# zuston/TonY

Measured on AMD Instinct MI355X. Metric: images/sec (whole node) Inception-v3 TF-PS, higher is better.
Workload: dtype bf16

## Files before the change

tony_amd/ops/csrc/conv.hip:

```cpp
#include <atomic>
#include <algorithm>
#include <cstdlib>
#include <type_traits>

#include "igemm.h"

using namespace tony;
using namespace tony::mfma;
using namespace tony::glds;

namespace tony {
int run_band(const Gather& g, const void* B, void* C, int64_t ldc, int64_t N, int epi, float* st, int64_t sstride,
             hipStream_t stream);
}

namespace {

__device__ __forceinline__ uint4 gather16(const Gather& g, const RowState& rs, const TapPos& t, int toff) {
  const int iy = rs.iy0 + g.sign * t.r, ix = rs.ix0 + g.sign * t.s;
  if (rs.ok && t.r < g.R && static_cast<unsigned>(iy) < static_cast<unsigned>(g.Hs) &&
      static_cast<unsigned>(ix) < static_cast<unsigned>(g.Ws))
    return *reinterpret_cast<const uint4*>(rs.base + toff);
  return make_uint4(0, 0, 0, 0);
}
// ... 602 lines not shown
  if (stats == nullptr) {
    stats = bnr.dsum;
    sstride = bnr.sstride;
  }
  float* st = stats + shard_off(blockIdx.x, sstride);
#pragma unroll
  for (int c = 0; c < D::CB; ++c)
#pragma unroll
    for (int r = 0; r < 4; ++r) {
      float a = ssum[c][r], q = ssq[c][r];
#pragma unroll
      for (int o = 1; o < 16; o <<= 1) {
        a += __shfl_xor(a, o, 64);
        q += __shfl_xor(q, o, 64);
      }
      if ((lane & 15) == 0) {
        atomicAdd(st + c * 16 + kq * 4 + r, a);
        atomicAdd(st + CO + c * 16 + kq * 4 + r, q);
      }
    }
}

int run_direct(const Gather& g, const void* B, void* C, int64_t ldc, int64_t N, int epi, float* st, int64_t sstride,
               hipStream_t stream, const BnRed& bnr = BnRed{}) {
  const bool f32 = (epi & 8) != 0;
  if (g.R != 3 || g.S != 3 || g.sh != 1 || g.sw != 1 || (epi & 22) || (ldc % 4) || g.halo_images <= 0 ||
      (reinterpret_cast<uintptr_t>(C) & (f32 ? 15 : 7)) || (reinterpret_cast<uintptr_t>(B) & 15) ||
      (f32 && bnr.z != nullptr))
    return -3;
  const auto launch = [&](auto cs, auto co, auto tw, auto f32c) -> int {
    constexpr int CS = decltype(cs)::value, CO = decltype(co)::value, TW = decltype(tw)::value;
    constexpr bool F32 = decltype(f32c)::value;
    using D = DirectCfg<CS, CO, TW>;
    const void* fn = reinterpret_cast<const void*>(&conv_direct_kernel<CS, CO, TW, F32>);
    static int per_cu = 0;
    if (per_cu == 0) {
      if (D::kLds > 65536 &&
          hipFuncSetAttribute(fn, hipFuncAttributeMaxDynamicSharedMemorySize, static_cast<int>(D::kLds)) != hipSuccess)
        return -3;
      if (hipOccupancyMaxActiveBlocksPerMultiprocessor(&per_cu, fn, kThreads, D::kLds) != hipSuccess || per_cu <= 0)
        per_cu = -1;
    }
    if (per_cu < 0) return -3;
    int dev = 0, cus = 0;
    if (hipGetDevice(&dev) != hipSuccess || hipDeviceGetAttribute(&cus, hipDeviceAttributeMultiprocessorCount, dev) !=
                                                hipSuccess)
      return -3;
    const int tiles_x = ceil_div(g.OW, TW), tiles_y = ceil_div(g.OH, kDirH);
    const int64_t ntiles = static_cast<int64_t>(g.halo_images) * tiles_x * tiles_y;
    if (ntiles > 0x7fffffff) return -2;
    const int grid = static_cast<int>(std::min<int64_t>(ntiles, static_cast<int64_t>(per_cu) * cus));
    conv_direct_kernel<CS, CO, TW, F32><<<grid, kThreads, D::kLds, stream>>>(
        g, static_cast<const uint16_t*>(B), static_cast<uint16_t*>(C), ldc, st, sstride, tiles_x, tiles_y,
        static_cast<int>(ntiles), bnr);
    TONY_LAUNCH_CHECK();
    return 0;
  };
  using I = std::integral_constant<int, 32>;
  using I64 = std::integral_constant<int, 64>;
  using I96 = std::integral_constant<int, 96>;
  using I16 = std::integral_constant<int, 16>;
  using BF = std::false_type;
  if (f32) {
    if (g.Cs == 96 && N == 32) return launch(I96{}, I{}, I{}, std::true_type{});
    if (g.Cs == 96 && N == 64) return launch(I96{}, I64{}, I16{}, std::true_type{});
    return -3;
  }
  if (g.Cs == 32 && N == 32) return launch(I{}, I{}, I{}, BF{});
  if (g.Cs == 32 && N == 64) return launch(I{}, I64{}, I16{}, BF{});
  if (g.Cs == 64 && N == 32) return launch(I64{}, I{}, I16{}, BF{});
  if (g.Cs == 64 && N == 64) return launch(I64{}, I64{}, I16{}, BF{});
  return -3;
}

int run_nt(const Gather& g, const void* B, void* C, int64_t ldc, int64_t M, int64_t N, int flags, float* stats,
           int64_t sstride, hipStream_t stream, const Phase& bph = Phase{}) {
  const int epi = flags & 31;
  if ((epi & 1) && (epi & 2)) return -1;
  if ((epi & 3) && stats == nullptr) return -1;
  if ((epi & 16) && ((epi & 3) || bph.bnr.z != nullptr)) return -1;
  float* st = stats;
  const int v = (flags >> 8) & 0xff;
  if (((flags >> 16) & 15) && !(v >= kGldsFirst && v < kGldsFirst + kNumGlds)) return -3;
  if (((epi & 24) && v == kHaloVariant) || ((epi & 16) && v == kDirectVariant)) return -3;
  if (v == kHaloVariant) return bph.bnr.z != nullptr ? -3 : run_halo(g, B, C, ldc, N, epi, st, sstride, stream);
  if (v == kBandVariant) return bph.bnr.z != nullptr ? -3 : run_band(g, B, C, ldc, N, epi, st, sstride, stream);
  if (v == kDirectVariant) return run_direct(g, B, C, ldc, N, epi, st, sstride, stream, bph.bnr);
  if (v >= kGldsFirst && v < kGldsFirst + kNumGlds)
    return bph.bnr.z != nullptr ? -3
                                : run_glds(g, B, g.K, C, ldc, M, N, epi, st, sstride, v, stream, RowMap{}, BTaps{},
                                           (flags >> 16) & 15);
  if (v >= kNumNtVariants) return -1;
  if (v == 0) {
    const int64_t bn = pick_bn(N, 192);
    return bn <= 64 ? launch_nt_bm<256>(g, B, C, ldc, M, N, st, sstride, epi, bn, stream, bph)
                    : launch_nt_bm<128>(g, B, C, ldc, M, N, st, sstride, epi, bn, stream, bph);
  }
  const int64_t bn = pick_bn(N, kNtVariants[v].cap);
  switch (kNtVariants[v].bm) {
    case 64: return launch_nt_bm<64>(g, B, C, ldc, M, N, st, sstride, epi, bn, stream, bph);
    case 128: return launch_nt_bm<128>(g, B, C, ldc, M, N, st, sstride, epi, bn, stream, bph);
    default: return launch_nt_bm<256>(g, B, C, ldc, M, N, st, sstride, epi, bn, stream, bph);
  }
}

int run_nt_phase(const Gather& g, const void* B, void* C, int64_t ldc, int64_t M, int64_t N, int v, const Phase& ph,
                 hipStream_t stream, int epi = 0) {
  if (v >= kGldsFirst && ph.bnr.z != nullptr) v = 0;
  if (v >= kGldsFirst)
    return run_glds(g, B, static_cast<int64_t>(ph.R) * ph.S * g.Cs, C, ldc, M, N, epi, nullptr, 0, v, stream, ph.rows,
                    BTaps{ph.r0, ph.s0, ph.tsy, ph.tsx, ph.S});
  if (v == kBandVariant) return -3;
  if (v == kHaloVariant || v == kDirectVariant || v >= kNumNtVariants) return -1;
  if (v == 0) {
    const int64_t bn = pick_bn(N, 192);
    return bn <= 64 ? launch_nt_bm<256, true>(g, B, C, ldc, M, N, nullptr, 0, epi, bn, stream, ph)
                    : launch_nt_bm<128, true>(g, B, C, ldc, M, N, nullptr, 0, epi, bn, stream, ph);
  }
  const int64_t bn = pick_bn(N, kNtVariants[v].cap);
  switch (kNtVariants[v].bm) {
    case 64: return launch_nt_bm<64, true>(g, B, C, ldc, M, N, nullptr, 0, epi, bn, stream, ph);
    case 128: return launch_nt_bm<128, true>(g, B, C, ldc, M, N, nullptr, 0, epi, bn, stream, ph);
    default: return launch_nt_bm<256, true>(g, B, C, ldc, M, N, nullptr, 0, epi, bn, stream, ph);
  }
}

constexpr int WTBM = 128;
constexpr int WTBN = 128;

struct MRow {
  int n, oy, ox;
  int64_t m;
  __device__ __forceinline__ void init(int64_t m_, const Gather& g) {
    m = m_;
    const int ohw = g.OH * g.OW;
    n = static_cast<int>(m_ / ohw);
    const int rem = static_cast<int>(m_ - static_cast<int64_t>(n) * ohw);
    oy = rem / g.OW;
    ox = rem - oy * g.OW;
  }
  __device__ __forceinline__ void advance(int dm, const Gather& g) {
    m += dm;
    ox += dm;
    while (ox >= g.OW) {
      ox -= g.OW;
      if (++oy == g.OH) {
        oy = 0;
        ++n;
      }
    }
  }
};

constexpr int WK = 32;

struct WkStep {
  int dx, dy, de;
  int cx, cy, ce;
  int img_y, img_e;
};

struct IncRows {
  int ix[2], iy[2], ie[2];
  int xlim, ylim;
  __device__ __forceinline__ void init(const MRow* mr, const Gather& g, const TapPos& tp) {
    xlim = g.OW * g.sw + g.offw + tp.s;
// ... 832 lines not shown
    case 96: ring == 3 ? go(std::integral_constant<int, 96>{}, I3{}) : go(std::integral_constant<int, 96>{}, I2{}); break;
    default: ring == 3 ? go(std::integral_constant<int, 128>{}, I3{}) : go(std::integral_constant<int, 128>{}, I2{}); break;
  }
  TONY_LAUNCH_CHECK();
  return 0;
}

int wgrad_tbm(int Co) {
  static const bool t96 = [] {
    const char* e = getenv("TONY_WGRAD_TBM96");
    return e == nullptr || e[0] != '0';
  }();
  if (Co <= 32) return 32;
  if (Co <= 64) return 64;
  return t96 && ceil_div(Co, 96) * 96 < ceil_div(Co, 128) * 128 ? 96 : 128;
}

bool bad_geom(int C, int64_t ld, const void* p) {
  return C <= 0 || (C % 8) || (ld % 8) || (reinterpret_cast<uintptr_t>(p) & 15);
}

}

namespace tony {
SplitWs& splitk_ws() {
  static thread_local SplitWs ws;
  return ws;
}
}

TONY_API int tony_splitk_workspace(float* slab, int64_t slab_floats, unsigned* cnt, int64_t ncnt) {
  if (slab_floats < 0 || ncnt < 0 || (reinterpret_cast<uintptr_t>(slab) & 15)) return -1;
  tony::splitk_ws() = tony::SplitWs{slab, slab_floats, cnt, ncnt};
  return 0;
}

int run_x3(Gather g, const void* B, int Cx, void* C, int64_t ldc, int64_t M, int64_t N, int flags, float* stats,
           int64_t sstride, hipStream_t stream) {
  const int v = (flags >> 8) & 0xff;
  if (v < kX3First || v >= kX3First + kNumX3 || Cx % 3 || (Cx / 3) % 8) return -3;
  const int epi = flags & 31;
  if ((epi & 1) && (epi & 2)) return -1;
  if ((epi & 3) && stats == nullptr) return -1;
  if ((epi & 16) && (epi & 3)) return -1;
  const int cp = Cx / 3;
  g.Cs = cp;
  g.K = g.R * g.S * cp;
  return run_glds_x3(g, B, static_cast<int64_t>(g.R) * g.S * Cx, C, ldc, M, N, epi, stats, sstride, v, stream,
                        RowMap{}, BTaps{}, (flags >> 16) & 15, X3Planes{cp, 2 * cp, 3 * cp});
}

TONY_API int tony_conv_fwd(const void* x, int N, int H, int W, int C, int64_t ldx, const void* w, int Co, int R,
                           int S, int sh, int sw, int ph, int pw, void* y, int OH, int OW, int64_t ldy, int flags,
                           float* stats, int64_t sstride, hipStream_t stream) {
  if (bad_geom(C, ldx, x) || (reinterpret_cast<uintptr_t>(w) & 15) || Co <= 0 || R <= 0 || S <= 0 || sstride < 0)
    return -1;
  if (OH != (H + 2 * ph - R) / sh + 1 || OW != (W + 2 * pw - S) / sw + 1 || OH <= 0 || OW <= 0) return -1;
  const int64_t M = static_cast<int64_t>(N) * OH * OW;
  if (M > 0x7fffffff || static_cast<int64_t>(N) * H * W > 0x7fffffff) return -1;
  Gather g{static_cast<const uint16_t*>(x), ldx, H, W, C, OH, OW, R, S, sh, sw, -ph, -pw, 1, R * S * C, N};
  const int v = (flags >> 8) & 0xff;
  if (v >= kX3First && v < kX3First + kNumX3) return run_x3(g, w, C, y, ldy, M, Co, flags, stats, sstride, stream);
  return run_nt(g, w, y, ldy, M, Co, flags, stats, sstride, stream);
}

TONY_API int tony_conv_dgrad(const void* dy, int N, int OH, int OW, int Co, int64_t lddy, const void* wt, int C,
                             int R, int S, int ph, int pw, void* dx, int H, int W, int64_t lddx, int flags,
                             BnRed* bnr, hipStream_t stream) {
  if (bad_geom(Co, lddy, dy) || (reinterpret_cast<uintptr_t>(wt) & 15) || C <= 0) return -1;
  if (OH != H + 2 * ph - R + 1 || OW != W + 2 * pw - S + 1) return -1;
  const int64_t M = static_cast<int64_t>(N) * H * W;
  if (M > 0x7fffffff || static_cast<int64_t>(N) * OH * OW > 0x7fffffff) return -1;
  Gather g{static_cast<const uint16_t*>(dy), lddy, OH, OW, Co, H, W, R, S, 1, 1, ph, pw, -1, R * S * Co, N};
  Phase bph{};
  if (bnr != nullptr) {
    bnr->done = 0;
    if (bnr->z != nullptr) {
      if (bnr->mean == nullptr || bnr->invstd == nullptr || bnr->dsum == nullptr || (bnr->ldz % 8) ||
          (reinterpret_cast<uintptr_t>(bnr->z) & 15) || (C % 8))
        return -1;
      bph.bnr = *bnr;
    }
  }
  const int fl = flags & 0xfff18;
  if ((fl & 16) && bph.bnr.z != nullptr) return -1;
  const int v = (fl >> 8) & 0xff;
  if (v >= kX3First && v < kX3First + kNumX3)
    return bph.bnr.z != nullptr ? -3 : run_x3(g, wt, Co, dx, lddx, M, C, fl, nullptr, 0, stream);
  const int rc = run_nt(g, wt, dx, lddx, M, C, fl, nullptr, 0, stream, bph);
  if (rc == -3 && bph.bnr.z != nullptr)
    return run_nt(g, wt, dx, lddx, M, C, fl, nullptr, 0, stream);
  if (rc == 0 && bph.bnr.z != nullptr) bnr->done = 1;
  return rc;
}

static std::atomic<int>& dgrad_one_launch_flag() {
  static std::atomic<int> on{[] {
    const char* e = std::getenv("TONY_DGRAD_ONE_LAUNCH");
    return (e != nullptr && e[0] == '0') ? 0 : 1;
  }()};
  return on;
}
static bool dgrad_one_launch() { return dgrad_one_launch_flag().load(std::memory_order_relaxed) != 0; }
TONY_API int tony_wgrad_pf(int on) {
  const int prev = wgrad_pf_flag().load();
  if (on >= 0) wgrad_pf_flag().store(on ? 1 : 0);
  return prev;
}

TONY_API int tony_dgrad_one_launch(int on) {
  const int prev = dgrad_one_launch_flag().load();
  if (on >= 0) dgrad_one_launch_flag().store(on ? 1 : 0);
  return prev;
}

TONY_API int tony_conv_dgrad_strided(const void* dy, int N, int OH, int OW, int Co, int64_t lddy, const void* wt,
                                     int C, int R, int S, int sh, int sw, int ph, int pw, void* dx, int H, int W,
                                     int64_t lddx, int flags, BnRed* bnr, hipStream_t stream) {
  if (bad_geom(Co, lddy, dy) || (reinterpret_cast<uintptr_t>(wt) & 15) || C <= 0 || C % 8 || (lddx % 8) ||
      (reinterpret_cast<uintptr_t>(dx) & 15))
    return -1;
  BnRed br{};
  if (bnr != nullptr) {
    bnr->done = 0;
    if (bnr->z != nullptr) {
      if (bnr->mean == nullptr || bnr->invstd == nullptr || bnr->dsum == nullptr || (bnr->ldz % 8) ||
          (reinterpret_cast<uintptr_t>(bnr->z) & 15))
        return -1;
      br = *bnr;
    }
  }
  if (sh < 1 || sw < 1 || sh > 4 || sw > 4 || ph < 0 || pw < 0 || ph >= R || pw >= S) return -1;
  if (OH != (H + 2 * ph - R) / sh + 1 || OW != (W + 2 * pw - S) / sw + 1 || OH <= 0 || OW <= 0) return -1;
  if (static_cast<int64_t>(N) * H * W > 0x7fffffff || static_cast<int64_t>(N) * OH * OW > 0x7fffffff) return -1;
  const int v = (flags >> 8) & 0xff;
  const int acc = flags & 16;
  if (acc && br.z != nullptr) return -1;
  if ((flags >> 16) & 15) return -3;
  const bool one = v >= kGldsFirst && v < kGldsFirst + kNumGlds && br.z == nullptr && sh * sw <= kMaxClasses &&
                   Co % kGldsVariants[v - kGldsFirst].kb == 0 && dgrad_one_launch();
  MultiClass mc{};
  for (int py = 0; py < sh; ++py) {
    for (int px = 0; px < sw; ++px) {
      const int QH = H > py ? (H - py + sh - 1) / sh : 0, QW = W > px ? (W - px + sw - 1) / sw : 0;
      const int64_t M = static_cast<int64_t>(N) * QH * QW;
      if (M == 0) continue;
      const int r0 = (py + ph) % sh, s0 = (px + pw) % sw;
      int Ra = r0 < R ? (R - r0 + sh - 1) / sh : 0, Sb = s0 < S ? (S - s0 + sw - 1) / sw : 0;
      const int cy = (py + ph - r0) / sh, cx = (px + pw - s0) / sw;
      if (Ra == 0 || Sb == 0) {
        if (acc) continue;
        Ra = 0, Sb = 1;
      }
      Gather g{static_cast<const uint16_t*>(dy), lddy, OH, OW, Co, QH, QW, Ra, Sb, 1, 1, cy, cx, -1, Ra * Sb * Co, N};
      Phase phz{R, S, r0, s0, sh, sw, RowMap{}};
      phz.rows.qw = QW;
      phz.rows.qhw = QH * QW;
      phz.rows.W = W;
      phz.rows.HW = H * W;
      phz.rows.sy = sh;
      phz.rows.sx = sw;
      phz.rows.y0 = py;
      phz.rows.x0 = px;
      phz.bnr = br;
      if (one) {
        mc.c[mc.n++] = ClassDesc{g, phz.rows, BTaps{r0, s0, sh, sw, S}, static_cast<int>(M), 0};
        continue;
// ... 109 lines not shown
```

tony_amd/ops/csrc/gemm.hip:

```cpp
#include <type_traits>
#include <cstdlib>

#include "igemm.h"

using namespace tony;
using namespace tony::mfma;
using namespace tony::glds;

namespace {

template <int ROWS>
__device__ __forceinline__ void load_tile(uint4* regs, const uint16_t* __restrict__ G, int64_t ld, int row0,
                                          int nrows, int k0, int K) {
  constexpr int VEC = ROWS * BK / 8 / kThreads;
#pragma unroll
  for (int i = 0; i < VEC; ++i) {
    const int v = threadIdx.x + i * kThreads;
    const int row = v >> 3, ch = v & 7;
    const int gr = row0 + row, gk = k0 + ch * 8;
    if (gr < nrows && gk < K)
      regs[i] = *reinterpret_cast<const uint4*>(G + static_cast<int64_t>(gr) * ld + gk);
    else
      regs[i] = make_uint4(0, 0, 0, 0);
  }
// ... 69 lines not shown
#pragma unroll
        for (int j = 0; j < TN; ++j) acc[i][j] = __builtin_amdgcn_mfma_f32_16x16x32_bf16(af[i], bfr[j], acc[i][j], 0, 0, 0);
    }
    if (more) {
      uint16_t* An = smem + ((kt + 1) & 1) * (BM + BN) * BK;
      store_tile<BM>(An, ra);
      store_tile<BN>(An + BM * BK, rb);
    }
    __syncthreads();
  }

  const bool am = (epi & 32) != 0;
  nt_epilogue<BM, BN, TM, TN>(acc, smem, C, ldc, M, N, m0, n0,
                               (epi & 1) ? stats + shard_off(tm, sstride) : nullptr,
                               (epi & 2) ? stats : nullptr, (epi & 4) != 0, RowMap{}, (epi & 8) != 0,
                               (epi & 48) != 0, am ? reinterpret_cast<const uint16_t*>(stats) : nullptr,
                               am ? reinterpret_cast<const uint8_t*>(sstride) : nullptr);
}

template <int BM, int BN>
int launch(const void* A, int64_t lda, const void* B, int64_t ldb, void* C, int64_t ldc, int64_t M, int64_t N,
           int64_t K, float* stats, int64_t sstride, int epi, hipStream_t stream) {
  const int tiles_m = ceil_div(M, BM), tiles_n = ceil_div(N, BN);
  const int64_t tiles = static_cast<int64_t>(tiles_m) * tiles_n;
  if (tiles > 0x7fffffff) return -2;
  gemm_nt_kernel<BM, BN><<<static_cast<int>(tiles), kThreads, 0, stream>>>(
      static_cast<const uint16_t*>(A), lda, static_cast<const uint16_t*>(B), ldb, static_cast<uint16_t*>(C), ldc,
      static_cast<int>(M), static_cast<int>(N), static_cast<int>(K), stats, sstride, epi, tiles_n);
  TONY_LAUNCH_CHECK();
  return 0;
}

template <int BM>
int launch_bm(const void* A, int64_t lda, const void* B, int64_t ldb, void* C, int64_t ldc, int64_t M, int64_t N,
              int64_t K, float* st, int64_t sstride, int epi, int64_t bn, hipStream_t stream) {
  if constexpr (BM == 256) {
    if (bn <= 32) return launch<256, 32>(A, lda, B, ldb, C, ldc, M, N, K, st, sstride, epi, stream);
    if (bn <= 64) return launch<256, 64>(A, lda, B, ldb, C, ldc, M, N, K, st, sstride, epi, stream);
    return -3;
  } else {
    switch (bn) {
      case 32: return launch<BM, 32>(A, lda, B, ldb, C, ldc, M, N, K, st, sstride, epi, stream);
      case 64: return launch<BM, 64>(A, lda, B, ldb, C, ldc, M, N, K, st, sstride, epi, stream);
      case 96: return launch<BM, 96>(A, lda, B, ldb, C, ldc, M, N, K, st, sstride, epi, stream);
      case 128: return launch<BM, 128>(A, lda, B, ldb, C, ldc, M, N, K, st, sstride, epi, stream);
      case 160: return launch<BM, 160>(A, lda, B, ldb, C, ldc, M, N, K, st, sstride, epi, stream);
      default: return launch<BM, 192>(A, lda, B, ldb, C, ldc, M, N, K, st, sstride, epi, stream);
    }
  }
}

}

TONY_API int tony_gemm_bf16_bnact(const void* A, const void* B, void* C, int64_t M, int64_t N, int64_t K, int64_t lda,
                                  int64_t ldb, int64_t ldc, int flags, float* stats, int64_t sstride, const float* table,
                                  hipStream_t stream) {
  if (M <= 0 || N <= 0 || K <= 0 || sstride < 0 || table == nullptr) return -1;
  if ((K % 8) || (lda % 8) || (ldb % 8) || M > 0x7fffffff || N > 0x7fffffff) return -1;
  if ((reinterpret_cast<uintptr_t>(A) | reinterpret_cast<uintptr_t>(B)) & 15) return -1;
  const int epi = flags & 31;
  if (((epi & 1) && (epi & 2)) || ((epi & 16) && (epi & 3)) || ((epi & 3) && stats == nullptr)) return -1;
  X3Planes xp{};
  xp.atab = table;
  return run_glds(gemm_gather(A, lda, M, K), B, ldb, C, ldc, M, N, epi, stats, sstride, kGldsFirst + 1, stream,
                  RowMap{}, BTaps{}, 0, xp);
}

TONY_API int tony_gemm_bf16(const void* A, const void* B, void* C, int64_t M, int64_t N, int64_t K, int64_t lda,
                            int64_t ldb, int64_t ldc, int flags, float* stats, int64_t sstride, hipStream_t stream) {
  if (M <= 0 || N <= 0 || K <= 0 || sstride < 0) return -1;
  if ((K % 8) || (lda % 8) || (ldb % 8)) return -1;
  if (M > 0x7fffffff || N > 0x7fffffff) return -1;
  if ((reinterpret_cast<uintptr_t>(A) | reinterpret_cast<uintptr_t>(B)) & 15) return -1;
  const int epi = flags & 63;
  if ((epi & 1) && (epi & 2)) return -1;
  if ((epi & 16) && (epi & 3)) return -1;
  if ((epi & 32) && ((epi & 31) || stats == nullptr || sstride == 0 || (ldc % 8) ||
                     (reinterpret_cast<uintptr_t>(stats) & 15)))
    return -1;
  if ((epi & 3) && stats == nullptr) return -1;
  float* st = stats;
  const int v = (flags >> 8) & 0xff;
  if (((flags >> 16) & 15) && !(v >= kGldsFirst && v < kGldsFirst + kNumGlds)) return -3;
  if (v >= kGldsFirst && v < kGldsFirst + kNumGlds)
    return run_glds(gemm_gather(A, lda, M, K), B, ldb, C, ldc, M, N, epi, st, sstride, v, stream, RowMap{}, BTaps{},
                    (flags >> 16) & 15);
  if (v >= kNumNtVariants) return -1;
  if (v == 0) {
    if (N <= 64) return launch<256, 64>(A, lda, B, ldb, C, ldc, M, N, K, st, sstride, epi, stream);
    return launch<128, 128>(A, lda, B, ldb, C, ldc, M, N, K, st, sstride, epi, stream);
  }
  const int64_t bn = pick_bn(N, kNtVariants[v].cap);
  switch (kNtVariants[v].bm) {
    case 64: return launch_bm<64>(A, lda, B, ldb, C, ldc, M, N, K, st, sstride, epi, bn, stream);
    case 128: return launch_bm<128>(A, lda, B, ldb, C, ldc, M, N, K, st, sstride, epi, bn, stream);
    default: return launch_bm<256>(A, lda, B, ldb, C, ldc, M, N, K, st, sstride, epi, bn, stream);
  }
}

namespace {

constexpr int TBM = 128;
constexpr int TBN = 128;

__device__ __forceinline__ void tn_load(uint4* regs, const uint16_t* __restrict__ G, int64_t ld, int64_t m0,
                                        int64_t m1, int c0, int ncols) {
#pragma unroll
  for (int i = 0; i < 2; ++i) {
    const int v = threadIdx.x + i * kThreads;
    const int row = v >> 4, ch = v & 15;
    const int64_t gm = m0 + row;
    const int gc = c0 + ch * 8;
    if (gm < m1 && gc < ncols)
      regs[i] = *reinterpret_cast<const uint4*>(G + gm * ld + gc);
    else
      regs[i] = make_uint4(0, 0, 0, 0);
  }
}

__device__ __forceinline__ void tn_store(uint16_t* lds, const uint4* regs) {
#pragma unroll
  for (int i = 0; i < 2; ++i) {
    const int v = threadIdx.x + i * kThreads;
    const int row = v >> 4, ch = v & 15;
    *reinterpret_cast<uint4*>(lds + tr_off(row, ch)) = regs[i];
  }
}

constexpr int kTnStages = 3;

__global__ __launch_bounds__(kThreads) __attribute__((amdgpu_waves_per_eu(2, 2))) void gemm_tn_glds_kernel(
    const uint16_t* __restrict__ A, int64_t lda, const uint16_t* __restrict__ B, int64_t ldb, int64_t M, int N1,
    int N2, int tiles_n2, int ntiles, int64_t rows_per_split, float* __restrict__ slab, SplitFold fold) {
  constexpr int TILE = TBK * 128, STAGE = 2 * TILE;
  __shared__ __attribute__((aligned(16))) uint16_t smem[kTnStages * STAGE];
  const int wg = xcd_remap(blockIdx.x, gridDim.x);
  const int tile = wg % ntiles, split = wg / ntiles;
  const int t1 = tile / tiles_n2, t2 = tile % tiles_n2;
  const int n1_0 = t1 * TBM, n2_0 = t2 * TBN;
  const int64_t m_begin = static_cast<int64_t>(split) * rows_per_split;
  const int64_t m_end = min(M, m_begin + rows_per_split);
  const int lane = threadIdx.x & 63, wave = threadIdx.x >> 6;
  const int wm = wave >> 1, wn = wave & 1;

  const int r0 = threadIdx.x >> 4;
  const int ch = (threadIdx.x & 15) ^ tr_swz(r0);
  const bool aok = n1_0 + ch * 8 < N1, bok = n2_0 + ch * 8 < N2;
  const uint16_t* ap = A + n1_0 + ch * 8;
  const uint16_t* bp = B + n2_0 + ch * 8;
  int am = static_cast<int>(m_begin) + r0;
  const int mend = static_cast<int>(m_end);
  const uint16_t* apm = ap + (m_begin + r0) * lda;
  const uint16_t* bpm = bp + (m_begin + r0) * ldb;
  const int64_t astep = TBK * lda, bstep = TBK * ldb;
  const uint32_t base = __builtin_amdgcn_readfirstlane(lds_addr(smem) + (4 * wave) * 256);
  constexpr uint32_t kRow16 = 16 * 256, kStageB = STAGE * 2, kTileB = TILE * 2;
  auto issue = [&](int slot) {
    const uint32_t As = base + slot * kStageB, Bs = As + kTileB;
    const void* z = &kZeroChunk;
#pragma unroll
    for (int i = 0; i < 2; ++i) {
      const bool mok = am + 16 * i < mend;
      glds16(aok & mok ? static_cast<const void*>(apm + i * 16 * lda) : z, As + i * kRow16);
      glds16(bok & mok ? static_cast<const void*>(bpm + i * 16 * ldb) : z, Bs + i * kRow16);
    }
    am += TBK;
// ... 197 lines not shown
```

tony_amd/ops/csrc/igemm.h:

```cpp
#pragma once

#include <algorithm>
#include <cstdlib>
#include <tuple>
#include <type_traits>

#include "mfma_common.h"

namespace tony {
struct SplitWs {
  float* slab = nullptr;
  int64_t slab_floats = 0;
  unsigned* cnt = nullptr;
  int64_t ncnt = 0;
};
SplitWs& splitk_ws();
}

namespace tony {
namespace glds {

using namespace tony::mfma;

struct SplitK {
// ... 572 lines not shown
    if (threadIdx.x == 0) {
      for (unsigned spins = 0; __hip_atomic_load(done, __ATOMIC_RELAXED, __HIP_MEMORY_SCOPE_AGENT) < others &&
                               spins < (1u << 24);
           ++spins)
        __builtin_amdgcn_s_sleep(1);
      __hip_atomic_store(cnt, 0u, __ATOMIC_RELAXED, __HIP_MEMORY_SCOPE_AGENT);
      __hip_atomic_store(done, 0u, __ATOMIC_RELAXED, __HIP_MEMORY_SCOPE_AGENT);
    }
    __syncthreads();
    __builtin_amdgcn_fence(__ATOMIC_ACQUIRE, "wavefront");
    f32x4 own[TM][TN];
#pragma unroll
    for (int i = 0; i < TM; ++i)
#pragma unroll
      for (int j = 0; j < TN; ++j) {
        own[i][j] = acc[i][j];
        acc[i][j] = f32x4{0.f, 0.f, 0.f, 0.f};
      }
    for (int c = w_first; c <= w_last; ++c) {
      if (c == w) {
#pragma unroll
        for (int i = 0; i < TM; ++i)
#pragma unroll
          for (int j = 0; j < TN; ++j) acc[i][j] += own[i][j];
        continue;
      }
      const int slot_c = (2 * c + ((static_cast<int64_t>(c) * T / G) >= t0 ? 0 : 1)) * FR;
#pragma unroll
      for (int i = 0; i < TM; ++i)
#pragma unroll
        for (int j = 0; j < TN; ++j)
          acc[i][j] += __builtin_bit_cast(f32x4, __builtin_amdgcn_raw_buffer_load_b128(
                                                     prs, ((slot_c + i * TN + j) * NT + threadIdx.x) * 16, 0, 16));
    }
  }
  const bool am = (epi & 32) != 0;
  nt_epilogue<BM, BN, TM, TN, ST * STAGE, NWM>(acc, smem, C, ldc, M, N, m0, n0,
                                           (epi & 1) ? stats + shard_off(tm, sstride) : nullptr,
                                           (epi & 2) ? stats : nullptr, (epi & 4) != 0, rmap, (epi & 8) != 0,
                                           (epi & 48) != 0, am ? reinterpret_cast<const uint16_t*>(stats) : nullptr,
                                           am ? reinterpret_cast<const uint8_t*>(sstride) : nullptr);
  if constexpr (!(FT & 1)) break;
  }
}

#define TONY_GLDS_PARAMS                                                                                      \
  Gather g, const uint16_t* __restrict__ B, int64_t ldb, uint16_t* __restrict__ C, int64_t ldc, int M, int N,   \
      float* __restrict__ stats, int64_t sstride, int epi, int tiles_n, RowMap rmap, BTaps bt, SplitK sk,       \
      X3Planes xp, MultiClass mc
#define TONY_GLDS_ARGS g, B, ldb, C, ldc, M, N, stats, sstride, epi, tiles_n, rmap, bt, sk, xp, mc
template <int BM, int BN, int ST, int KB, bool UNI, int NWM = 2, bool IL = false, bool X3 = false, bool AT = false,
          bool PF = false, int FT = 0>
__global__ __launch_bounds__(128 * NWM) void conv_glds_kernel(TONY_GLDS_PARAMS) {
  conv_glds_body<BM, BN, ST, KB, UNI, NWM, IL, X3, AT, PF, FT>(TONY_GLDS_ARGS);
}
template <int BM, int BN, int ST, int KB, bool UNI, int NWM, bool IL, int WPE, int FT = 0>
__global__ __launch_bounds__(128 * NWM) __attribute__((amdgpu_waves_per_eu(WPE))) void conv_glds_occ_kernel(
    TONY_GLDS_PARAMS) {
  conv_glds_body<BM, BN, ST, KB, UNI, NWM, IL, false, false, false, FT>(TONY_GLDS_ARGS);
}
#undef TONY_GLDS_PARAMS
#undef TONY_GLDS_ARGS

constexpr int64_t kStreamMaxTiles = 4096;
inline int num_cus_of_current() {
  static int cached[16] = {0};
  int dev = 0;
  if (hipGetDevice(&dev) != hipSuccess || dev < 0 || dev >= 16) return 256;
  if (cached[dev] == 0) {
    int n = 0;
    cached[dev] = hipDeviceGetAttribute(&n, hipDeviceAttributeMultiprocessorCount, dev) == hipSuccess && n > 0 ? n : 256;
  }
  return cached[dev];
}

struct X3Variant {
  int bm, cap, stages, kb, nwm;
};
constexpr int kX3First = 32;
constexpr X3Variant kX3Variants[] = {{256, 128, 2, 32, 4}, {128, 192, 3, 32, 2}, {128, 128, 4, 32, 2},
                                     {128, 128, 2, 64, 2}, {256, 128, 3, 32, 4}, {64, 128, 4, 32, 2}};
constexpr int kNumX3 = sizeof(kX3Variants) / sizeof(kX3Variants[0]);

constexpr int glds_part(int c) { return c <= 4 ? 0 : c <= 8 ? 1 : c <= 13 ? 2 : 3; }

int run_glds(const Gather& g, const void* B, int64_t ldb, void* C, int64_t ldc, int64_t M, int64_t N, int epi,
             float* st, int64_t sstride, int v, hipStream_t stream, RowMap rmap = RowMap{}, BTaps bt = BTaps{},
             int stream_m = 0, X3Planes xp = X3Planes{}, const MultiClass* classes = nullptr);
int run_glds_x3(const Gather& g, const void* B, int64_t ldb, void* C, int64_t ldc, int64_t M, int64_t N, int epi,
                float* st, int64_t sstride, int v, hipStream_t stream, RowMap rmap, BTaps bt, int stream_m,
                X3Planes xp);
template <bool XF, int PART>
int run_glds_part(const Gather& g, const void* B, int64_t ldb, void* C, int64_t ldc, int64_t M, int64_t N, int epi,
                  float* st, int64_t sstride, int v, hipStream_t stream, RowMap rmap, BTaps bt, int stream_m,
                  X3Planes xp, const MultiClass* classes);

}
}
```

tony_amd/ops/tune.py:

```python
from __future__ import annotations

import os
from typing import Callable, Dict, Hashable

import torch

AUTOTUNE = os.environ.get("TONY_CONV_AUTOTUNE", "1") != "0"
_N_GLDS = (25 if os.environ.get("TONY_CONV_GLDS_IL", "1") != "0" else 20) \
    if os.environ.get("TONY_CONV_GLDS8", "1") != "0" else 16
_BASE = tuple(range(_N_GLDS if os.environ.get("TONY_CONV_GLDS", "1") != "0" else 11))
if os.environ.get("TONY_CONV_OCC", "1") != "0" and os.environ.get("TONY_CONV_GLDS", "1") != "0":
    _BASE = _BASE + tuple(range(25, 32))
STREAM_MS = tuple(int(x) for x in os.environ.get("TONY_STREAMK", "").split(",") if x.strip() not in ("", "0"))
NT_VARIANTS = _BASE + tuple(v + 256 * m for m in STREAM_MS for v in _BASE if v >= 11)
BAND_CODE = 40
CONV_VARIANTS = NT_VARIANTS + ((BAND_CODE,) if os.environ.get("TONY_CONV_BAND", "0") == "1" else ())
X3_STREAM_MS = tuple(int(x) for x in os.environ.get("TONY_X3_STREAMK", "1").split(",") if x.strip() not in ("", "0"))
X3F_CODES = tuple(range(32, 38)) if os.environ.get("TONY_X3_FUSED", "1") != "0" else ()
X3_VARIANTS = _BASE + tuple(v + 256 * m for m in X3_STREAM_MS for v in _BASE if v >= 11)
X3F_VARIANTS = X3F_CODES + tuple(v + 256 * m for m in X3_STREAM_MS for v in X3F_CODES)
SMALL_GEMM_VARIANTS = _BASE + tuple(v + 256 * m for m in (1, 2) for v in _BASE if v >= 11)


def stream_of(vflags: int) -> int:
    return (vflags >> 16) & 15
_CACHE: Dict[Hashable, int] = {}


def time_ms(fn: Callable[[], object], reps: int = 5) -> float:
    fn()
    torch.cuda.synchronize()
    start, end = torch.cuda.Event(enable_timing=True), torch.cuda.Event(enable_timing=True)
    torch.cuda._sleep(4_000_000)
    start.record()
    for _ in range(reps):
        fn()
    end.record()
    end.synchronize()
    return start.elapsed_time(end) / reps


def pick(key: Hashable, launch: Callable[[int], int], variants=NT_VARIANTS) -> int:
    v = _CACHE.get(key)
    if v is not None:
        return v << 8
    if not AUTOTUNE or torch.cuda.is_current_stream_capturing():
        return 0
    best, best_t = 0, float("inf")
    for cand in variants:
        if launch(cand << 8) != 0:
            continue
        t = time_ms(lambda: launch(cand << 8))
        if t < best_t:
            best, best_t = cand, t
    _CACHE[key] = best
    return best << 8


def pick_choice(key: Hashable, choices, run: Callable[[object], object]):
    c = _CACHE.get(key)
    if c is not None:
        return c
    if not AUTOTUNE or torch.cuda.is_current_stream_capturing():
        return choices[0]
    times = {ch: time_ms(lambda: run(ch)) for ch in choices}
    best = min(times, key=times.get)
    _CACHE[key] = best
    return best


def cached(key: Hashable):
    v = _CACHE.get(key)
    if v is not None:
        return v << 8
    if not AUTOTUNE or torch.cuda.is_current_stream_capturing():
        return 0
    return None


def choices() -> Dict[Hashable, int]:
    return dict(_CACHE)


def gemm_flags(a: torch.Tensor, b: torch.Tensor, c: torch.Tensor, M: int, N: int, K: int, lda: int,
               stats: bool, variants=NT_VARIANTS) -> int:
    from . import _lib

    key = ("gemm", M, N, K, lda, bool(stats))
    if key in _CACHE or not AUTOTUNE or torch.cuda.is_current_stream_capturing():
        return pick(key, lambda vf: 0)
    L = _lib.lib()
    dev = c.device
    stream = _lib.stream_ptr(dev)
    scratch = torch.zeros(_lib.stat_floats(N), dtype=torch.float32, device=dev)
    base = 1 if stats else 0
    return pick(key, lambda vf: L.tony_gemm_bf16(a.data_ptr(), b.data_ptr(), c.data_ptr(), M, N, K, lda, K, N,
                                                 base | vf, scratch.data_ptr(), 2 * N, stream), variants)
# ... 28 lines not shown
```

Measured before the change: 9428.

## Add wave-quantization-fitted GLDS tile variants to the autotuned conv and GEMM set

After: 9536, median of 3. No clear change (+1.1%).

```diff
diff --git a/tony_amd/ops/csrc/conv.hip b/tony_amd/ops/csrc/conv.hip
--- a/tony_amd/ops/csrc/conv.hip
+++ b/tony_amd/ops/csrc/conv.hip
@@ -708,6 +708,10 @@
   float* st = stats;
   const int v = (flags >> 8) & 0xff;
   if (((flags >> 16) & 15) && !(v >= kGldsFirst && v < kGldsFirst + kNumGlds)) return -3;
+  if (is_fit(v))
+    return bph.bnr.z != nullptr
+               ? -3
+               : run_glds_fit(g, B, g.K, C, ldc, M, N, epi, st, sstride, v, stream, (flags & kFitForce) != 0);
   if (((epi & 24) && v == kHaloVariant) || ((epi & 16) && v == kDirectVariant)) return -3;
   if (v == kHaloVariant) return bph.bnr.z != nullptr ? -3 : run_halo(g, B, C, ldc, N, epi, st, sstride, stream);
   if (v == kBandVariant) return bph.bnr.z != nullptr ? -3 : run_band(g, B, C, ldc, N, epi, st, sstride, stream);
@@ -1706,7 +1710,7 @@
       bph.bnr = *bnr;
     }
   }
-  const int fl = flags & 0xfff18;
+  const int fl = flags & 0x1fff18;
   if ((fl & 16) && bph.bnr.z != nullptr) return -1;
   const int v = (fl >> 8) & 0xff;
   if (v >= kX3First && v < kX3First + kNumX3)
diff --git a/tony_amd/ops/csrc/gemm.hip b/tony_amd/ops/csrc/gemm.hip
--- a/tony_amd/ops/csrc/gemm.hip
+++ b/tony_amd/ops/csrc/gemm.hip
@@ -175,6 +175,9 @@
   float* st = stats;
   const int v = (flags >> 8) & 0xff;
   if (((flags >> 16) & 15) && !(v >= kGldsFirst && v < kGldsFirst + kNumGlds)) return -3;
+  if (is_fit(v))
+    return run_glds_fit(gemm_gather(A, lda, M, K), B, ldb, C, ldc, M, N, epi, st, sstride, v, stream,
+                        (flags & kFitForce) != 0);
   if (v >= kGldsFirst && v < kGldsFirst + kNumGlds)
     return run_glds(gemm_gather(A, lda, M, K), B, ldb, C, ldc, M, N, epi, st, sstride, v, stream, RowMap{}, BTaps{},
                     (flags >> 16) & 15);
diff --git a/tony_amd/ops/csrc/glds_fit.hip b/tony_amd/ops/csrc/glds_fit.hip
--- /dev/null
+++ b/tony_amd/ops/csrc/glds_fit.hip
@@ -0,0 +1,99 @@
+#include "igemm.h"
+
+namespace tony {
+namespace glds {
+
+namespace {
+
+struct FitArgs {
+  const Gather& g;
+  const uint16_t* B;
+  int64_t ldb;
+  uint16_t* C;
+  int64_t ldc;
+  int64_t M, N;
+  int epi;
+  float* st;
+  int64_t sstride;
+  hipStream_t stream;
+  bool force;
+};
+
+template <int CODE, int BN>
+int launch_fit(const FitArgs& a) {
+  constexpr GldsVariant T = kFitVariants[CODE - kFitFirst];
+  constexpr int BM = T.bm, ST = T.stages, KB = T.kb, NWM = T.nwm, WPE = T.wpe;
+  constexpr int RING = ST * (BM + BN) * KB;
+  constexpr int RES = fit_resident(T, BN);
+  if constexpr (RES < (WPE > 0 ? WPE * 2 / NWM : 1)) {
+    return -3;
+  } else {
+    static_assert(T.il && !T.pf && KB == 32, "fitted tiles: 32-deep stages, interleaved issue");
+    static_assert((BM / NWM) % 16 == 0 && BM % NWM == 0, "a wave's rows are whole 16-row MFMA tiles");
+    static_assert(BM % (64 / (KB / 8)) == 0 && BN % (64 / (KB / 8)) == 0 && BN % 32 == 0, "whole DMA row groups");
+    static_assert(BM * (BN + 8) <= RING, "the epilogue's C tile fits in the ring");
+    static_assert(RING * 2 * RES <= kLdsBytes && RES >= 1, "the resident workgroups' rings fit the LDS");
+    if (!a.force && !fit_applies(a.M, a.N, BM, BN, num_cus_of_current(), RES)) return -3;
+    const int tiles_n = ceil_div(a.N, BN);
+    const int64_t tiles = static_cast<int64_t>(ceil_div(a.M, BM)) * tiles_n;
+    if (tiles > 0x7fffffff) return -2;
+    const int grid = static_cast<int>(tiles);
+    const int M = static_cast<int>(a.M), N = static_cast<int>(a.N);
+    if constexpr (WPE > 0)
+      conv_glds_occ_kernel<BM, BN, ST, KB, true, NWM, true, WPE, 0><<<grid, 128 * NWM, 0, a.stream>>>(
+          a.g, a.B, a.ldb, a.C, a.ldc, M, N, a.st, a.sstride, a.epi, tiles_n, RowMap{}, BTaps{}, SplitK{}, X3Planes{},
+          MultiClass{});
+    else
+      conv_glds_kernel<BM, BN, ST, KB, true, NWM, true, false, false, false, 0><<<grid, 128 * NWM, 0, a.stream>>>(
+          a.g, a.B, a.ldb, a.C, a.ldc, M, N, a.st, a.sstride, a.epi, tiles_n, RowMap{}, BTaps{}, SplitK{}, X3Planes{},
+          MultiClass{});
+    TONY_LAUNCH_CHECK();
+    return 0;
+  }
+}
+
+template <int CODE>
+int by_bn(const FitArgs& a) {
+  constexpr int CAP = kFitVariants[CODE - kFitFirst].cap;
+  switch (pick_bn(a.N, CAP)) {
+    case 32: return launch_fit<CODE, 32>(a);
+    case 64: return launch_fit<CODE, 64>(a);
+    case 96:
+      if constexpr (CAP >= 96) return launch_fit<CODE, 96>(a);
+      break;
+    case 128:
+      if constexpr (CAP >= 128) return launch_fit<CODE, 128>(a);
+      break;
+    case 160:
+      if constexpr (CAP >= 160) return launch_fit<CODE, 160>(a);
+      break;
+    case 192:
+      if constexpr (CAP >= 192) return launch_fit<CODE, 192>(a);
+      break;
+    default: break;
+  }
+  return -3;
+}
+
+template <int... I>
+int dispatch(int v, const FitArgs& a, std::integer_sequence<int, I...>) {
+  int rc = -3;
+  (void)((v == kFitFirst + I ? (rc = by_bn<kFitFirst + I>(a), true) : false) || ...);
+  return rc;
+}
+
+}
+
+int run_glds_fit(const Gather& g, const void* B, int64_t ldb, void* C, int64_t ldc, int64_t M, int64_t N, int epi,
+                 float* st, int64_t sstride, int v, hipStream_t stream, bool force) {
+  if ((ldc % 8) || (ldb % 8) || (reinterpret_cast<uintptr_t>(C) & 15) || (reinterpret_cast<uintptr_t>(B) & 15) ||
+      (reinterpret_cast<uintptr_t>(g.src) & 15) || (g.ld % 8) || (g.K % 8))
+    return -3;
+  if (!is_fit(v) || g.Cs % 32 != 0 || !glds_uni_enabled()) return -3;
+  const FitArgs a{g, static_cast<const uint16_t*>(B), ldb, static_cast<uint16_t*>(C), ldc, M, N, epi, st, sstride,
+                  stream, force};
+  return dispatch(v, a, std::make_integer_sequence<int, kNumFit>{});
+}
+
+}
+}
diff --git a/tony_amd/ops/csrc/igemm.h b/tony_amd/ops/csrc/igemm.h
--- a/tony_amd/ops/csrc/igemm.h
+++ b/tony_amd/ops/csrc/igemm.h
@@ -678,6 +678,29 @@
                                      {128, 128, 2, 64, 2}, {256, 128, 3, 32, 4}, {64, 128, 4, 32, 2}};
 constexpr int kNumX3 = sizeof(kX3Variants) / sizeof(kX3Variants[0]);
 
+constexpr int kFitFirst = 41;
+constexpr int kFitForce = 1 << 20;
+constexpr GldsVariant kFitVariants[] = {
+    {320, 128, 4, 32, 4, true}, {384, 128, 4, 32, 4, true}, {192, 128, 3, 32, 4, true, false, 4}};
+constexpr int kNumFit = sizeof(kFitVariants) / sizeof(kFitVariants[0]);
+constexpr int kLdsBytes = 163840;
+
+inline bool is_fit(int v) { return v >= kFitFirst && v < kFitFirst + kNumFit; }
+
+constexpr int fit_resident(const GldsVariant& t, int bn) {
+  const int by_lds = kLdsBytes / (t.stages * (t.bm + bn) * t.kb * 2);
+  const int by_waves = t.wpe > 0 ? t.wpe * 2 / t.nwm : (t.nwm == 4 ? 1 : 2);
+  return by_lds < by_waves ? by_lds : by_waves;
+}
+constexpr int64_t fit_rounds(int64_t M, int64_t N, int bm, int bn, int cus, int resident) {
+  const int64_t wgs = ((M + bm - 1) / bm) * ((N + bn - 1) / bn), slots = static_cast<int64_t>(cus) * resident;
+  return (wgs + slots - 1) / slots;
+}
+constexpr bool fit_applies(int64_t M, int64_t N, int bm, int bn, int cus, int resident) {
+  const int64_t rf = fit_rounds(M, N, bm, bn, cus, resident), r256 = fit_rounds(M, N, 256, bn, cus, resident);
+  return rf < r256 || (bm < 256 && rf == r256);
+}
+
 constexpr int glds_part(int c) { return c <= 4 ? 0 : c <= 8 ? 1 : c <= 13 ? 2 : 3; }
 
 int run_glds(const Gather& g, const void* B, int64_t ldb, void* C, int64_t ldc, int64_t M, int64_t N, int epi,
@@ -686,6 +709,8 @@
 int run_glds_x3(const Gather& g, const void* B, int64_t ldb, void* C, int64_t ldc, int64_t M, int64_t N, int epi,
                 float* st, int64_t sstride, int v, hipStream_t stream, RowMap rmap, BTaps bt, int stream_m,
                 X3Planes xp);
+int run_glds_fit(const Gather& g, const void* B, int64_t ldb, void* C, int64_t ldc, int64_t M, int64_t N, int epi,
+                 float* st, int64_t sstride, int v, hipStream_t stream, bool force);
 template <bool XF, int PART>
 int run_glds_part(const Gather& g, const void* B, int64_t ldb, void* C, int64_t ldc, int64_t M, int64_t N, int epi,
                   float* st, int64_t sstride, int v, hipStream_t stream, RowMap rmap, BTaps bt, int stream_m,
diff --git a/tony_amd/ops/tune.py b/tony_amd/ops/tune.py
--- a/tony_amd/ops/tune.py
+++ b/tony_amd/ops/tune.py
@@ -12,7 +12,34 @@
 if os.environ.get("TONY_CONV_OCC", "1") != "0" and os.environ.get("TONY_CONV_GLDS", "1") != "0":
     _BASE = _BASE + tuple(range(25, 32))
 STREAM_MS = tuple(int(x) for x in os.environ.get("TONY_STREAMK", "").split(",") if x.strip() not in ("", "0"))
-NT_VARIANTS = _BASE + tuple(v + 256 * m for m in STREAM_MS for v in _BASE if v >= 11)
+FIT_FIRST = 41
+FIT_FORCE = 1 << 20
+FIT_TILES = ((320, 128, 4, 4, 0), (384, 128, 4, 4, 0), (192, 128, 3, 4, 4))
+FIT_CODES = tuple(range(FIT_FIRST, FIT_FIRST + len(FIT_TILES))) \
+    if os.environ.get("TONY_CONV_FIT", "1") != "0" and os.environ.get("TONY_CONV_GLDS", "1") != "0" else ()
+NT_VARIANTS = _BASE + FIT_CODES + tuple(v + 256 * m for m in STREAM_MS for v in _BASE if v >= 11)
+
+
+def fit_bn(n: int, cap: int) -> int:
+    ntn = -(-n // cap)
+    return -(-(-(-n // ntn)) // 32) * 32
+
+
+def fit_resident(tile, bn: int) -> int:
+    bm, _, stages, nwm, wpe = tile
+    by_lds = 163840 // (stages * (bm + bn) * 32 * 2)
+    return min(by_lds, wpe * 2 // nwm if wpe else (1 if nwm == 4 else 2))
+
+
+def fit_rounds(m: int, n: int, bm: int, bn: int, cus: int, resident: int) -> int:
+    return -(-(-(-m // bm) * -(-n // bn)) // (cus * resident))
+
+
+def fit_applies(m: int, n: int, bm: int, bn: int, cus: int, resident: int) -> bool:
+    rf, r256 = fit_rounds(m, n, bm, bn, cus, resident), fit_rounds(m, n, 256, bn, cus, resident)
+    return rf < r256 or (bm < 256 and rf == r256)
+
+
 BAND_CODE = 40
 CONV_VARIANTS = NT_VARIANTS + ((BAND_CODE,) if os.environ.get("TONY_CONV_BAND", "0") == "1" else ())
 X3_STREAM_MS = tuple(int(x) for x in os.environ.get("TONY_X3_STREAMK", "1").split(",") if x.strip() not in ("", "0"))
```
